# MachinePerceptionLab/Attentive_DFPrior

Hardware: AMD Instinct MI355X
Metric: rendered rays/sec (64 samples/ray), Replica room0 (higher is better)
Workload: dtype f32 via f16x3 split (3 f16 MFMA products per f32 product: 22-bit products, f32 accumulate); 1 GPU; room0 640x480 render_img, 64 spp (48+16), synthetic box room, seed-0 random decoders, grids at the REFERENCE init (N(0,.01), high N(0,1e-4)); stage color, ray_batch_size 100000 (per-batch far clamp, rendered as one call with a depth maximum per 100 000-ray segment), ONE frame per step; samples_per_ray=64

## Files before the change

attentive_dfprior_amd/csrc/adfp_decode_g.h:

```cpp
#pragma once
#include "adfp_decode_h.h"

__host__ __device__ constexpr int unit16(int k) { return 16 * ((k & 7) >> 2) + 4 * (k >> 3) + (k & 3); }

template <int CDIM, int NOUT>
struct DecLayoutG {
    using F = DecLayout<CDIM, NOUT>;
    static constexpr int KG_E = 3;
    static constexpr int KG_C = CDIM / 32;
    __host__ __device__ static constexpr int kg(int i) { return i == 0 ? KG_E : (i == 3 ? KG_E + 1 : 1); }
    static constexpr int P_BM = 0;
    __host__ __device__ static constexpr int layer_words(int i) { return kg(i) * 1024 + 32 + KG_C * 1024 + 32; }
    __host__ __device__ static constexpr int P_WP(int i) {
        int o = 384;
        for (int k = 0; k < i; ++k) o += layer_words(k);
        return o;
    }
    __host__ __device__ static constexpr int P_BP(int i) { return P_WP(i) + kg(i) * 1024; }
    __host__ __device__ static constexpr int P_WC(int i) { return P_BP(i) + 32; }
    __host__ __device__ static constexpr int P_BC(int i) { return P_WC(i) + KG_C * 1024; }
    static constexpr int P_WO = P_WP(5);
    static constexpr int P_BO = P_WO + NOUT * 32;
    static constexpr int P_FLAG = P_BO + 4;
    static constexpr int NFLAG = (((P_FLAG + 511) / 256) + 3) & ~3;
    static constexpr int P_TOTAL = P_FLAG + NFLAG;
    static_assert((P_TOTAL + 255) / 256 <= NFLAG, "one flag word per pack block");
};

template <int CDIM, int NOUT>
__device__ HSrc dec_g_src(int t) {
    using L = DecLayoutG<CDIM, NOUT>;
    using F = DecLayout<CDIM, NOUT>;
    if (t < 384) {
        const int row = t >> 2, c = t & 3;
        const int f = (row & ~31) + unit16(row & 31);
        return HSrc{0, (f < 93 && c < 3) ? F::F_EB + c * 93 + f : -1, -1};
    }
#pragma unroll
    for (int i = 0; i < 5; ++i) {
        if (t < L::P_BP(i) || (t >= L::P_WC(i) && t < L::P_BC(i))) {
            const bool fc = t >= L::P_WC(i);
            const int u = t - (fc ? L::P_WC(i) : L::P_WP(i));
            const int grp = u >> 10, ob = (u >> 9) & 1, part = (u >> 8) & 1, g = (u >> 6) & 3, row = 16 * ob + ((u >> 2) & 15), jp = (u & 3) * 2;
            int src[2];
#pragma unroll
            for (int e = 0; e < 2; ++e) {
                int col = 32 * grp + unit16(8 * g + jp + e);
                if (fc) src[e] = F::F_FC(i) + row * CDIM + col;
                else {
                    if (i == 0) { if (col >= 93) col = -1; }
                    else if (i == 3) { if (col < 96) { if (col >= 93) col = -1; } else col = 93 + (col - 96); }
                    src[e] = col < 0 ? -1 : F::F_PL(i) + row * F::in_dim(i) + col;
                }
            }
            return HSrc{1 + part, src[0], src[1]};
        }
        if (t < L::P_WC(i)) return HSrc{0, F::F_PL(i) + 32 * F::in_dim(i) + (t - L::P_BP(i)), -1};
        if (t < L::P_BC(i) + 32) return HSrc{0, F::F_FC(i) + 32 * CDIM + (t - L::P_BC(i)), -1};
    }
    if (t < L::P_BO) {
        const int u = t - L::P_WO;
        return HSrc{0, F::F_OW + u, -1};
    }
    const int o = t - L::P_BO;
    return HSrc{0, o < NOUT ? F::F_OB + o : -1, -1};
}

template <int CDIM, int NOUT>
ADFP_DEV void pack_decoder_g_block(int blk, const float* __restrict__ flat, unsigned* __restrict__ packed, int* __restrict__ status, int bit) {
    using L = DecLayoutG<CDIM, NOUT>;
    const int t = blk * 256 + (int)threadIdx.x;
    HSrc s{0, -1, -1};
    float a = 0.f, b = 0.f;
    if (t < L::P_FLAG) {
        s = dec_g_src<CDIM, NOUT>(t);
        a = s.s0 < 0 ? 0.f : flat[s.s0]; b = s.s1 < 0 ? 0.f : flat[s.s1];
    }
    pack_block_flag(!(fmaxf(fabsf(a), fabsf(b)) < 65504.0f), packed + L::P_FLAG + blk, status, bit);
    if (t >= L::P_FLAG) return;
    if (s.kind == 0) { packed[t] = s.s0 < 0 ? 0u : __float_as_uint(a); return; }
    a = f16_clamp(a); b = f16_clamp(b);
    const float ah = f16_hi_part(a), bh = f16_hi_part(b);
    _Float16 x, y;
    if (s.kind == 1) { x = (_Float16)ah; y = (_Float16)bh; }
    else { x = (_Float16)(a - ah); y = (_Float16)(b - bh); }
    packed[t] = (unsigned)__builtin_bit_cast(unsigned short, x) | ((unsigned)__builtin_bit_cast(unsigned short, y) << 16);
}
template <int CDIM, int NOUT>
__global__ void k_pack_decoder_g(const float* __restrict__ flat, unsigned* __restrict__ packed, int* __restrict__ status, int bit) { pack_decoder_g_block<CDIM, NOUT>((int)blockIdx.x, flat, packed, status, bit); }

typedef float f32x4g __attribute__((ext_vector_type(4)));

ADFP_DEV void swap_halves(float& x, float& y) {
    const auto r = __builtin_amdgcn_permlane32_swap(__float_as_uint(x), __float_as_uint(y), false, false);
    x = __uint_as_float(r[0]); y = __uint_as_float(r[1]);
}

template <int NG>
ADFP_DEV void mfma_chain_g(f32x4g acc[2][2], const unsigned* __restrict__ w, const f16x8 (*xh)[2], const f16x8 (*xl)[2]) {
#pragma unroll
    for (int kg = 0; kg < NG; ++kg) {
#pragma unroll
        for (int ob = 0; ob < 2; ++ob) {
            const f16x8 ah = __builtin_bit_cast(f16x8, *(const u32x4*)(w + kg * 1024 + ob * 512));
            const f16x8 al = __builtin_bit_cast(f16x8, *(const u32x4*)(w + kg * 1024 + ob * 512 + 256));
#pragma unroll
            for (int pb = 0; pb < 2; ++pb) {
                acc[ob][pb] = __builtin_amdgcn_mfma_f32_16x16x32_f16(ah, xh[kg][pb], acc[ob][pb], 0, 0, 0);
                acc[ob][pb] = __builtin_amdgcn_mfma_f32_16x16x32_f16(ah, xl[kg][pb], acc[ob][pb], 0, 0, 0);
                acc[ob][pb] = __builtin_amdgcn_mfma_f32_16x16x32_f16(al, xh[kg][pb], acc[ob][pb], 0, 0, 0);
            }
        }
    }
    __builtin_amdgcn_sched_barrier(0);
}

ADFP_DEV void row_store(float* p, const f32x4 v) {
    *(f32x4*)p = v;
}
template <int CDIM, int NOUT, int TRAIN = 0>
ADFP_DEV void decode_net_g(const unsigned* __restrict__ ldsu, const GridDev& grid, const GridDev& grid1, const float pn[3], const float (*pf)[3],
                           int lane, float& amax, float (*out)[NOUT], unsigned* __restrict__ mw, float* srow0, unsigned rowbits) {
    using L = DecLayoutG<CDIM, NOUT>;
    using ST = DecStage<CDIM>;
    const int g = lane >> 4;
    float* srow[2] = {nullptr, nullptr};
    if constexpr (TRAIN) {
        srow[0] = (rowbits & 1u) ? srow0 : nullptr;
        srow[1] = (rowbits & 2u) ? srow0 + 16 * ST::NXM : nullptr;
    }
    const unsigned* wl = ldsu + 4 * lane;
    const float* b4 = (const float*)ldsu + 4 * g;
    const float* brow = (const float*)ldsu + 32 * g;
    f16x8 ch[L::KG_C][2], cl[L::KG_C][2];
#pragma unroll
    for (int kc = 0; kc < L::KG_C; ++kc) {
        float c[16];
        gather16(kc == 0 ? grid : grid1, pn, g & 1, c);
        float x[8] = {c[0], c[1], c[2], c[3], c[8], c[9], c[10], c[11]};
        float y[8] = {c[4], c[5], c[6], c[7], c[12], c[13], c[14], c[15]};
#pragma unroll
        for (int s = 0; s < 8; ++s) swap_halves(x[s], y[s]);
        if constexpr (TRAIN) {
            static_assert(!TRAIN || CDIM == 32, "training rows: 32-channel decoders");
            if (srow[0]) { row_store(srow[0] + ST::xm(ST::SC) + 4 * g, f32x4{x[0], x[1], x[2], x[3]}); row_store(srow[0] + ST::xm(ST::SC) + 16 + 4 * g, f32x4{x[4], x[5], x[6], x[7]}); }
            if (srow[1]) { row_store(srow[1] + ST::xm(ST::SC) + 4 * g, f32x4{y[0], y[1], y[2], y[3]}); row_store(srow[1] + ST::xm(ST::SC) + 16 + 4 * g, f32x4{y[4], y[5], y[6], y[7]}); }
        }
        split8(x, ch[kc][0], cl[kc][0], amax);
        split8(y, ch[kc][1], cl[kc][1], amax);
    }
    f16x8 eh[L::KG_E][2], el[L::KG_E][2];
#pragma unroll
    for (int kg = 0; kg < L::KG_E; ++kg) {
        float e0[8], e1[8];
#pragma unroll
        for (int j = 0; j < 8; ++j) {
            const f32x4 bm = *(const f32x4*)(brow + L::P_BM + (32 * kg + j) * 4);
            e0[j] = adfp_sinf(fmaf(pf[0][2], bm.z, fmaf(pf[0][1], bm.y, pf[0][0] * bm.x)));
            e1[j] = adfp_sinf(fmaf(pf[1][2], bm.z, fmaf(pf[1][1], bm.y, pf[1][0] * bm.x)));
        }
        split8<false>(e0, eh[kg][0], el[kg][0], amax);
        split8<false>(e1, eh[kg][1], el[kg][1], amax);
    }
    __builtin_amdgcn_sched_barrier(0);
    f32x4g acc[2][2];
    f16x8 hh[1][2], hl[1][2];
    unsigned mk[3] = {0u, 0u, 0u};
#pragma unroll
    for (int i = 0; i < 5; ++i) {
#pragma unroll
        for (int ob = 0; ob < 2; ++ob) { const f32x4 t = *(const f32x4*)(b4 + L::P_BP(i) + 16 * ob); acc[ob][0] = t; acc[ob][1] = t; }
        if (i == 0) mfma_chain_g<L::KG_E>(acc, wl + L::P_WP(0), eh, el);
        else if (i == 3) {
            mfma_chain_g<L::KG_E>(acc, wl + L::P_WP(3), eh, el);
            mfma_chain_g<1>(acc, wl + L::P_WP(3) + L::KG_E * 1024, hh, hl);
        } else mfma_chain_g<1>(acc, wl + L::P_WP(i), hh, hl);
#pragma unroll
        for (int ob = 0; ob < 2; ++ob) {
            const f32x4 t = *(const f32x4*)(b4 + L::P_BC(i) + 16 * ob);
#pragma unroll
            for (int pb = 0; pb < 2; ++pb)
#pragma unroll
                for (int r = 0; r < 4; ++r) {
                    const float v = relu_f(acc[ob][pb][r]);
                    if constexpr (TRAIN) mk[i >> 1] = __builtin_amdgcn_alignbit(mk[i >> 1], 0u - __float_as_uint(v), 31);
                    acc[ob][pb][r] = v + t[r];
                }
        }
        mfma_chain_g<L::KG_C>(acc, wl + L::P_WC(i), ch, cl);
        if constexpr (TRAIN) {
#pragma unroll
            for (int pb = 0; pb < 2; ++pb) if (srow[pb]) {
                row_store(srow[pb] + ST::xm(ST::SH(i)) + 4 * g, f32x4{acc[0][pb][0], acc[0][pb][1], acc[0][pb][2], acc[0][pb][3]});
                row_store(srow[pb] + ST::xm(ST::SH(i)) + 16 + 4 * g, f32x4{acc[1][pb][0], acc[1][pb][1], acc[1][pb][2], acc[1][pb][3]});
            }
        }
        if (i < 4) {
#pragma unroll
            for (int pb = 0; pb < 2; ++pb) {
                const float t[8] = {acc[0][pb][0], acc[0][pb][1], acc[0][pb][2], acc[0][pb][3],
                                    acc[1][pb][0], acc[1][pb][1], acc[1][pb][2], acc[1][pb][3]};
                split8(t, hh[0][pb], hl[0][pb], amax);
            }
        }
    }
#pragma unroll
    for (int o = 0; o < NOUT; ++o) {
        const f32x4 w0 = *(const f32x4*)(b4 + L::P_WO + 32 * o), w1 = *(const f32x4*)(b4 + L::P_WO + 32 * o + 16);
#pragma unroll
        for (int pb = 0; pb < 2; ++pb) {
            float s = 0.f;
#pragma unroll
            for (int r = 0; r < 4; ++r) s = fmaf(acc[0][pb][r], w0[r], s);
#pragma unroll
            for (int r = 0; r < 4; ++r) s = fmaf(acc[1][pb][r], w1[r], s);
            s += __shfl_xor(s, 16);
            s += __shfl_xor(s, 32);
            out[pb][o] = s + ((const float*)ldsu)[L::P_BO + o];
        }
    }
    if constexpr (TRAIN) {
        const int sh = 4 * (g >> 1);
        unsigned wpb[2][3];
#pragma unroll
        for (int pb = 0; pb < 2; ++pb) {
            unsigned f[5];
#pragma unroll
            for (int i = 0; i < 5; ++i) {
                const unsigned m16 = (i == 4 || (i & 1)) ? (mk[i >> 1] & 0xFFFFu) : (mk[i >> 1] >> 16);
                const unsigned n0 = (m16 >> (12 - 4 * pb)) & 0xFu, n1 = (m16 >> (4 - 4 * pb)) & 0xFu;
                f[i] = (n0 << (12 - sh)) | (n1 << (4 - sh));
            }
            wpb[pb][0] = f[0] | (f[1] << 16); wpb[pb][1] = f[2] | (f[3] << 16); wpb[pb][2] = f[4];
        }
#pragma unroll
        for (int k = 0; k < 3; ++k) {
            const auto r = __builtin_amdgcn_permlane32_swap(wpb[0][k], wpb[1][k], false, false);
            mw[k] = r[0] | r[1];
        }
    }
}

template <int NT>
__global__ __launch_bounds__(NT, NT / 256) void k_decode_lc16(DecodeLCArgs a) {
    using LL = DecLayoutG<32, 1>;
    using LC = DecLayoutG<32, 4>;
    __shared__ __attribute__((aligned(16))) unsigned lds_all[LL::P_TOTAL + LC::P_TOTAL];
    __shared__ int s_next;
    __shared__ unsigned long long s_ring[ADFP_POOL_RING];
    unsigned* lds_low = lds_all;
    unsigned* lds_col = lds_all + LL::P_TOTAL;
    image_to_lds<NT, LL::P_TOTAL / 4>(lds_low, a.packed_low);
    image_to_lds<NT, LC::P_TOTAL / 4>(lds_col, a.packed_color);
    if (threadIdx.x == 0) s_next = NT / 64;
    if (threadIdx.x < ADFP_POOL_RING) s_ring[threadIdx.x] = 0ull;
    __syncthreads();
    const int lane = threadIdx.x & 63, n = lane & 15, g = lane >> 4;
    const int count = a.P.n;
    const int ntiles = (count + 31) >> 5;
    const TilePlan plan = tile_plan(ntiles, (int)gridDim.x, NT / 64, a.pool != nullptr);
    float amax_low = image_out_of_range<LL::P_FLAG, LL::NFLAG>(lds_low) ? INFINITY : 0.f;
    float amax_col = image_out_of_range<LC::P_FLAG, LC::NFLAG>(lds_col) ? INFINITY : 0.f;
    for (int j = threadIdx.x >> 6, tile; (tile = claim_tile_pool<NT / 64>(j, &s_next, s_ring, plan, ntiles, a.pool, a.status)) >= 0;) {
        const int idx = tile * 32 + 16 * (g >> 1) + n;
        const bool valid = idx < count;
        const int q = valid ? idx : 0;
        float pn[3], pf[2][3];
        bool pnan, keep_occ;
        {
            double pt[3];
            load_point(a.P, q, pt);
            normalize3(a.nb, pt, pn);
            const float f0 = (float)pt[0], f1 = (float)pt[1], f2 = (float)pt[2];
            pnan = (pt[0] != pt[0]) | (pt[1] != pt[1]) | (pt[2] != pt[2]);
            const unsigned f = a.flags ? a.flags[q] : 0u;
            keep_occ = (f & ADFP_F_BAND) || in_bound(pt, a.b) || !a.apply_bound;
            pf[0][0] = f0; pf[0][1] = f1; pf[0][2] = f2; pf[1][0] = f0; pf[1][1] = f1; pf[1][2] = f2;
        }
#pragma unroll
        for (int k = 0; k < 3; ++k) swap_halves(pf[0][k], pf[1][k]);
        float occ[2][1], rgb[2][4];
        int off_low = 0, off_col = LL::P_TOTAL;
        asm volatile("" : "+v"(off_low), "+v"(off_col));
        decode_net_g<32, 1>(lds_all + off_low, a.g_low, a.g_low, pn, pf, lane, amax_low, occ, nullptr, nullptr, 0u);
        asm volatile("" : "+v"(pn[0]), "+v"(pn[1]), "+v"(pn[2]), "+v"(occ[0][0]), "+v"(occ[1][0]));
        __builtin_amdgcn_sched_barrier(0);
        decode_net_g<32, 4>(lds_all + off_col, a.g_color, a.g_color, pn, pf, lane, amax_col, rgb, nullptr, nullptr, 0u);
        if (valid && (g & 1) == 0) {
            const int pb = g >> 1;
            const float nanv = __builtin_nanf("");
            const float o = pnan ? nanv : (keep_occ ? (pb ? occ[1][0] : occ[0][0]) : 100.f);
            const f32x4 c4 = pb ? f32x4{rgb[1][0], rgb[1][1], rgb[1][2], o} : f32x4{rgb[0][0], rgb[0][1], rgb[0][2], o};
            *(f32x4*)(a.raw + 4ll * q) = pnan ? f32x4{nanv, nanv, nanv, o} : c4;
            if (a.write_w) a.w[q] = 1.f;
        }
    }
    report_range(a.status, amax_low, ADFP_STATUS_F16_RANGE_LOW, a.call_flag);
    report_range(a.status, amax_col, ADFP_STATUS_F16_RANGE_COLOR, a.call_flag);
}

struct DecodeLCTrainArgs {
    DecodeLCArgs f;
    unsigned* masks_low; unsigned* masks_color;
    float* act_low; float* act_color;
    int split_networks;
};
template <int NT, bool SPLIT = false>
__global__ __launch_bounds__(NT, NT / 256) void k_decode_lc16_train(DecodeLCTrainArgs t) {
    const DecodeLCArgs& a = t.f;
    using LL = DecLayoutG<32, 1>;
    using LC = DecLayoutG<32, 4>;
    using ST = DecStage<32>;
    __shared__ __attribute__((aligned(16))) unsigned lds_all[LL::P_TOTAL + LC::P_TOTAL];
    __shared__ int s_next;
    unsigned* lds_low = lds_all;
    unsigned* lds_col = lds_all + LL::P_TOTAL;
    image_to_lds<NT, LL::P_TOTAL / 4>(lds_low, a.packed_low);
    image_to_lds<NT, LC::P_TOTAL / 4>(lds_col, a.packed_color);
    if (threadIdx.x == 0) s_next = NT / 64;
    __syncthreads();
    const int lane = threadIdx.x & 63, n = lane & 15, g = lane >> 4;
    const int count = a.P.n;
    const int ntiles = (count + 31) >> 5;
    float amax_low = image_out_of_range<LL::P_FLAG, LL::NFLAG>(lds_low) ? INFINITY : 0.f;
    float amax_col = image_out_of_range<LC::P_FLAG, LC::NFLAG>(lds_col) ? INFINITY : 0.f;
    constexpr bool split = SPLIT;
    const int njobs = split ? 2 * ntiles : ntiles;
    for (int j = threadIdx.x >> 6, job; (job = claim_tile<NT / 64>(j, &s_next, njobs)) >= 0;) {
        const int tile = split ? job >> 1 : job;
        const bool do_low = !split || (job & 1) == 0, do_col = !split || (job & 1) == 1;
        const int idx = tile * 32 + 16 * (g >> 1) + n;
        const bool valid = idx < count;
        const int q = valid ? idx : 0;
        float pn[3], pf[2][3];
        bool pnan, keep_occ;
        {
            double pt[3];
            load_point(a.P, q, pt);
            normalize3(a.nb, pt, pn);
            pnan = (pt[0] != pt[0]) | (pt[1] != pt[1]) | (pt[2] != pt[2]);
            const float f0 = pnan ? 0.f : (float)pt[0], f1 = pnan ? 0.f : (float)pt[1], f2 = pnan ? 0.f : (float)pt[2];
            const unsigned f = a.flags ? a.flags[q] : 0u;
            keep_occ = (f & ADFP_F_BAND) || in_bound(pt, a.b) || !a.apply_bound;
            pf[0][0] = f0; pf[0][1] = f1; pf[0][2] = f2; pf[1][0] = f0; pf[1][1] = f1; pf[1][2] = f2;
        }
#pragma unroll
        for (int k = 0; k < 3; ++k) swap_halves(pf[0][k], pf[1][k]);
        const int i0 = tile * 32 + n;
        const unsigned rowbits = (i0 < count ? 1u : 0u) | (i0 + 16 < count ? 2u : 0u);
        float occ[2][1], rgb[2][4];
        unsigned mw[3];
        int off_low = 0, off_col = LL::P_TOTAL;
        asm volatile("" : "+v"(off_low), "+v"(off_col));
        if constexpr (split) {
            occ[0][0] = 0.f; occ[1][0] = 0.f;
#pragma unroll
            for (int k = 0; k < 4; ++k) { rgb[0][k] = 0.f; rgb[1][k] = 0.f; }
        }
        if (do_low) {
            decode_net_g<32, 1, 1>(lds_all + off_low, a.g_low, a.g_low, pn, pf, lane, amax_low, occ, mw, t.act_low + (long long)i0 * ST::NXM, t.act_low ? rowbits : 0u);
            if (valid) { unsigned* mrow = t.masks_low + ((long long)q * 2 + (g & 1)) * 3; mrow[0] = mw[0]; mrow[1] = mw[1]; mrow[2] = mw[2]; }
        }
        asm volatile("" : "+v"(pn[0]), "+v"(pn[1]), "+v"(pn[2]), "+v"(occ[0][0]), "+v"(occ[1][0]));
        __builtin_amdgcn_sched_barrier(0);
        if (do_col) {
            decode_net_g<32, 4, 1>(lds_all + off_col, a.g_color, a.g_color, pn, pf, lane, amax_col, rgb, mw, t.act_color + (long long)i0 * ST::NXM, t.act_color ? rowbits : 0u);
            if (valid) { unsigned* mrow = t.masks_color + ((long long)q * 2 + (g & 1)) * 3; mrow[0] = mw[0]; mrow[1] = mw[1]; mrow[2] = mw[2]; }
        }
        if (valid && (g & 1) == 0) {
            const int pb = g >> 1;
            const float nanv = __builtin_nanf("");
            const float o = pnan ? nanv : (keep_occ ? (pb ? occ[1][0] : occ[0][0]) : 100.f);
            const f32x4 c4 = pb ? f32x4{rgb[1][0], rgb[1][1], rgb[1][2], o} : f32x4{rgb[0][0], rgb[0][1], rgb[0][2], o};
            const f32x4 row = pnan ? f32x4{nanv, nanv, nanv, o} : c4;
            if (!split) {
                *(f32x4*)(a.raw + 4ll * q) = row;
                if (a.write_w) a.w[q] = 1.f;
            } else if (do_low) {
                a.raw[4ll * q + 3] = row.w;
                if (a.write_w) a.w[q] = 1.f;
            } else {
                a.raw[4ll * q] = row.x; a.raw[4ll * q + 1] = row.y; a.raw[4ll * q + 2] = row.z;
            }
        }
    }
    report_range(a.status, amax_low, ADFP_STATUS_F16_RANGE_LOW, a.call_flag);
    report_range(a.status, amax_col, ADFP_STATUS_F16_RANGE_COLOR, a.call_flag);
}

template <int NT>
__global__ __launch_bounds__(NT, NT / 256) void k_decode_high_g(DecodeArgs a) {
    using L = DecLayoutG<64, 1>;
    __shared__ __attribute__((aligned(16))) unsigned ldsu[L::P_TOTAL];
    __shared__ int s_next;
    __shared__ unsigned long long s_ring[ADFP_POOL_RING];
    image_to_lds<NT, L::P_TOTAL / 4>(ldsu, a.packed);
    if (threadIdx.x == 0) s_next = NT / 64;
    if (threadIdx.x < ADFP_POOL_RING) s_ring[threadIdx.x] = 0ull;
    __syncthreads();
    const int lane = threadIdx.x & 63, n = lane & 15, g = lane >> 4;
    const int count = *a.count_ptr;
    const int ntiles = (count + 31) >> 5;
    const TilePlan plan = tile_plan(ntiles, (int)gridDim.x, NT / 64, a.pool != nullptr);
    float amax = image_out_of_range<L::P_FLAG, L::NFLAG>(ldsu) ? INFINITY : 0.f;
    for (int j = threadIdx.x >> 6, tile; (tile = claim_tile_pool<NT / 64>(j, &s_next, s_ring, plan, ntiles, a.pool, a.status)) >= 0;) {
        const int idx = tile * 32 + 16 * (g >> 1) + n;
        const bool valid = idx < count;
        const int q = a.list[valid ? idx : 0];
        float pn[3], pf[2][3];
        bool pnan;
        const float low_occ = (a.single || !valid) ? 0.f : a.raw[4ll * q + 3];
        {
            double pt[3];
            load_point(a.P, q, pt);
            normalize3(a.nb, pt, pn);
            const float f0 = (float)pt[0], f1 = (float)pt[1], f2 = (float)pt[2];
            pnan = (pt[0] != pt[0]) | (pt[1] != pt[1]) | (pt[2] != pt[2]);
            pf[0][0] = f0; pf[0][1] = f1; pf[0][2] = f2; pf[1][0] = f0; pf[1][1] = f1; pf[1][2] = f2;
        }
#pragma unroll
        for (int k = 0; k < 3; ++k) swap_halves(pf[0][k], pf[1][k]);
        float out[2][1];
        decode_net_g<64, 1>(ldsu, a.g0, a.g1, pn, pf, lane, amax, out, nullptr, nullptr, 0u);
        if (valid && (g & 1) == 0) {
            const float o = g >> 1 ? out[1][0] : out[0][0];
            const float v = pnan ? __builtin_nanf("") : o;
            a.att_occ[idx] = a.single ? v : v + low_occ;
        }
    }
    report_range(a.status, amax, ADFP_STATUS_F16_RANGE_HIGH, a.call_flag);
}

struct AttLayoutG {
    using F = AttLayout;
    static constexpr int P_A0 = 0;
    static constexpr int P_W1 = 256;
    static constexpr int P_B1 = P_W1 + 4 * 2 * 1024;
    static constexpr int P_W2 = P_B1 + 128;
    static constexpr int P_B2 = P_W2 + 4 * 4 * 1024;
    static constexpr int P_W3 = P_B2 + 128;
    static constexpr int P_B3 = P_W3 + 2 * 4 * 1024;
    static constexpr int P_WO = P_B3 + 64;
    static constexpr int P_BO = P_WO + 128;
    static constexpr int P_FLAG = P_BO + 4;
    static constexpr int NFLAG = (((P_FLAG + 511) / 256) + 3) & ~3;
    static constexpr int P_TOTAL = P_FLAG + NFLAG;
    static_assert((P_TOTAL + 255) / 256 <= NFLAG, "one flag word per pack block");
};

__device__ HSrc att_g_src(int t) {
    using L = AttLayoutG;
    using F = AttLayout;
    if (t < L::P_W1) {
        const int row = t >> 2, c = t & 3;
        const int u = (row & ~31) + unit16(row & 31);
        return HSrc{0, c < 2 ? F::F_W0 + u * 2 + c : (c == 2 ? F::F_B0 + u : -1), -1};
    }
    auto chain = [](int u, int ngrp, int base, int ld) {
        const int blk = u / (ngrp * 1024), v = u % (ngrp * 1024);
        const int grp = v >> 10, ob = (v >> 9) & 1, part = (v >> 8) & 1, g = (v >> 6) & 3, row = 32 * blk + 16 * ob + ((v >> 2) & 15), jp = (v & 3) * 2;
        return HSrc{1 + part, base + row * ld + 32 * grp + unit16(8 * g + jp), base + row * ld + 32 * grp + unit16(8 * g + jp + 1)};
    };
    if (t < L::P_B1) return chain(t - L::P_W1, 2, F::F_W1, 64);
    if (t < L::P_W2) return HSrc{0, F::F_B1 + (t - L::P_B1), -1};
    if (t < L::P_B2) return chain(t - L::P_W2, 4, F::F_W2, 128);
    if (t < L::P_W3) return HSrc{0, F::F_B2 + (t - L::P_B2), -1};
    if (t < L::P_B3) return chain(t - L::P_W3, 4, F::F_W3, 128);
    if (t < L::P_WO) return HSrc{0, F::F_B3 + (t - L::P_B3), -1};
    if (t < L::P_BO) return HSrc{0, F::F_WO + (t - L::P_WO), -1};
    const int o = t - L::P_BO;
    return HSrc{0, o < 2 ? F::F_BO + o : -1, -1};
}

ADFP_DEV void pack_attention_g_block(int blk, const float* __restrict__ flat, unsigned* __restrict__ packed, int* __restrict__ status) {
    using L = AttLayoutG;
    const int t = blk * 256 + (int)threadIdx.x;
    HSrc s{0, -1, -1};
    float a = 0.f, b = 0.f;
    if (t < L::P_FLAG) {
        s = att_g_src(t);
        a = s.s0 < 0 ? 0.f : flat[s.s0]; b = s.s1 < 0 ? 0.f : flat[s.s1];
    }
    pack_block_flag(!(fmaxf(fabsf(a), fabsf(b)) < 65504.0f), packed + L::P_FLAG + blk, status, ADFP_STATUS_F16_RANGE_ATT);
    if (t >= L::P_FLAG) return;
    if (s.kind == 0) { packed[t] = s.s0 < 0 ? 0u : __float_as_uint(a); return; }
    a = f16_clamp(a); b = f16_clamp(b);
    const float ah = f16_hi_part(a), bh = f16_hi_part(b);
    _Float16 x, y;
    if (s.kind == 1) { x = (_Float16)ah; y = (_Float16)bh; }
    else { x = (_Float16)(a - ah); y = (_Float16)(b - bh); }
    packed[t] = (unsigned)__builtin_bit_cast(unsigned short, x) | ((unsigned)__builtin_bit_cast(unsigned short, y) << 16);
}
__global__ void k_pack_attention_g(const float* __restrict__ flat, unsigned* __restrict__ packed, int* __restrict__ status) { pack_attention_g_block((int)blockIdx.x, flat, packed, status); }

template <int NT>
__global__ __launch_bounds__(NT) void k_attention_g(AttArgs a) {
    using A = AttLayoutG;
    __shared__ __attribute__((aligned(16))) unsigned ldsu[A::P_TOTAL];
    __shared__ int s_next;
    __shared__ unsigned long long s_ring[ADFP_POOL_RING];
    image_to_lds<NT, A::P_TOTAL / 4>(ldsu, a.packed);
    if (threadIdx.x == 0) s_next = NT / 64;
    if (threadIdx.x < ADFP_POOL_RING) s_ring[threadIdx.x] = 0ull;
    __syncthreads();
    const float* lds = (const float*)ldsu;
    const int lane = threadIdx.x & 63, n = lane & 15, g = lane >> 4;
    const unsigned* wl = ldsu + 4 * lane;
    const float* b4 = lds + 4 * g;
    const float* arow = lds + 32 * g;
    const int count = a.count_ptr ? *a.count_ptr : a.n_rows;
    const int ntiles = (count + 31) >> 5;
    const TilePlan plan = tile_plan(ntiles, (int)gridDim.x, NT / 64, a.pool != nullptr);
    float amax = image_out_of_range<A::P_FLAG, A::NFLAG>(ldsu) ? INFINITY : 0.f;
    for (int j = threadIdx.x >> 6, tile; (tile = claim_tile_pool<NT / 64>(j, &s_next, s_ring, plan, ntiles, a.pool, a.status)) >= 0;) {
        int idx[2]; bool valid[2]; float occ[2], u[2];
#pragma unroll
        for (int pb = 0; pb < 2; ++pb) {
            idx[pb] = tile * 32 + 16 * pb + n;
            valid[pb] = idx[pb] < count;
            const int ii = valid[pb] ? idx[pb] : 0;
            occ[pb] = a.att_occ[ii]; u[pb] = a.att_u[ii];
        }
        f16x8 xh[4][2], xl[4][2];
#pragma unroll
        for (int b = 0; b < 2; ++b) {
            float t0[8], t1[8];
#pragma unroll
            for (int k = 0; k < 8; ++k) {
                const f32x4 t = *(const f32x4*)(arow + A::P_A0 + (32 * b + k) * 4);
                t0[k] = relu_f(fmaf(u[0], t.y, fmaf(occ[0], t.x, t.z)));
                t1[k] = relu_f(fmaf(u[1], t.y, fmaf(occ[1], t.x, t.z)));
            }
            split8(t0, xh[b][0], xl[b][0], amax);
            split8(t1, xh[b][1], xl[b][1], amax);
        }
        __builtin_amdgcn_sched_barrier(0);
        f16x8 yh[4][2], yl[4][2];
#pragma unroll
        for (int blk = 0; blk < 4; ++blk) {
            f32x4g acc[2][2];
#pragma unroll
            for (int ob = 0; ob < 2; ++ob) { const f32x4 t = *(const f32x4*)(b4 + A::P_B1 + 32 * blk + 16 * ob); acc[ob][0] = t; acc[ob][1] = t; }
            mfma_chain_g<2>(acc, wl + A::P_W1 + blk * 2 * 1024, xh, xl);
#pragma unroll
            for (int pb = 0; pb < 2; ++pb) {
                const float t[8] = {relu_f(acc[0][pb][0]), relu_f(acc[0][pb][1]), relu_f(acc[0][pb][2]), relu_f(acc[0][pb][3]),
                                    relu_f(acc[1][pb][0]), relu_f(acc[1][pb][1]), relu_f(acc[1][pb][2]), relu_f(acc[1][pb][3])};
                split8(t, yh[blk][pb], yl[blk][pb], amax);
            }
        }
#pragma unroll
        for (int blk = 0; blk < 4; ++blk) {
            f32x4g acc[2][2];
#pragma unroll
            for (int ob = 0; ob < 2; ++ob) { const f32x4 t = *(const f32x4*)(b4 + A::P_B2 + 32 * blk + 16 * ob); acc[ob][0] = t; acc[ob][1] = t; }
            mfma_chain_g<4>(acc, wl + A::P_W2 + blk * 4 * 1024, yh, yl);
#pragma unroll
            for (int pb = 0; pb < 2; ++pb) {
                const float t[8] = {relu_f(acc[0][pb][0]), relu_f(acc[0][pb][1]), relu_f(acc[0][pb][2]), relu_f(acc[0][pb][3]),
                                    relu_f(acc[1][pb][0]), relu_f(acc[1][pb][1]), relu_f(acc[1][pb][2]), relu_f(acc[1][pb][3])};
                split8(t, xh[blk][pb], xl[blk][pb], amax);
            }
        }
        float l0[2] = {0.f, 0.f}, l1[2] = {0.f, 0.f};
#pragma unroll
        for (int blk = 0; blk < 2; ++blk) {
            f32x4g acc[2][2];
#pragma unroll
            for (int ob = 0; ob < 2; ++ob) { const f32x4 t = *(const f32x4*)(b4 + A::P_B3 + 32 * blk + 16 * ob); acc[ob][0] = t; acc[ob][1] = t; }
            mfma_chain_g<4>(acc, wl + A::P_W3 + blk * 4 * 1024, xh, xl);
#pragma unroll
            for (int ob = 0; ob < 2; ++ob) {
                const f32x4 w0 = *(const f32x4*)(b4 + A::P_WO + 32 * blk + 16 * ob), w1 = *(const f32x4*)(b4 + A::P_WO + 64 + 32 * blk + 16 * ob);
#pragma unroll
                for (int pb = 0; pb < 2; ++pb)
#pragma unroll
                    for (int r = 0; r < 4; ++r) {
                        const float v = relu_f(acc[ob][pb][r]);
                        l0[pb] = fmaf(v, w0[r], l0[pb]);
                        l1[pb] = fmaf(v, w1[r], l1[pb]);
                    }
            }
        }
#pragma unroll
        for (int pb = 0; pb < 2; ++pb) {
            l0[pb] += __shfl_xor(l0[pb], 16); l0[pb] += __shfl_xor(l0[pb], 32);
            l1[pb] += __shfl_xor(l1[pb], 16); l1[pb] += __shfl_xor(l1[pb], 32);
        }
        if (g < 2 && valid[g]) {
            const float a0l = l0[g] + lds[A::P_BO], a1l = l1[g] + lds[A::P_BO + 1];
            const float m = fmaxf(a0l, a1l);
            const float e0 = expf(a0l - m), e1 = expf(a1l - m);
            const float den = e0 + e1;
            const float a0 = e0 / den, a1 = e1 / den;
            const float fused = a0 * occ[g] + a1 * u[g];
            const int ii = idx[g];
            const int q = a.list ? a.list[ii] : ii;
            const bool inb = !a.flags || (a.flags[q] & ADFP_F_INBOUND) != 0;
            a.raw[4ll * q + 3] = (inb || !a.apply_bound) ? fused : 100.f;
            a.w[q] = a1;
        }
    }
    report_range(a.status, amax, ADFP_STATUS_F16_RANGE_ATT, a.call_flag);
}
```

Measured before the change: 58.87 million rays/s.

## Software-pipeline high decoder and attention MLP chains with interleaved LDS reads and MFMA

Adds a hand-scheduled high-band decoder (decode_net_gp) that double-buffers weight operand reads from LDS and interleaves the Fourier feature computation, ReLU and f16 splitting with MFMA chains, using sched_group_barrier slots. The attention kernel is rewritten into one flattened 10-chunk chain. It prefetches the next chunk's weights and the next tile's inputs while the current MFMAs run, and spreads the previous chunk's epilogue (split or output dot) between MFMAs. The aim is to hide LDS latency and VALU epilogue work behind matrix ops, at the cost of higher register pressure and fragile compiler scheduling.

```diff
diff --git a/attentive_dfprior_amd/csrc/adfp_decode_g.h b/attentive_dfprior_amd/csrc/adfp_decode_g.h
--- a/attentive_dfprior_amd/csrc/adfp_decode_g.h
+++ b/attentive_dfprior_amd/csrc/adfp_decode_g.h
@@ -388,6 +388,210 @@
     report_range(a.status, amax_col, ADFP_STATUS_F16_RANGE_COLOR, a.call_flag);
 }
 
+struct AOpG { u32x4 h[2], l[2]; };
+ADFP_DEV void aop_read(AOpG& A, const unsigned* __restrict__ w, int ob) {
+    A.h[ob] = *(const u32x4*)(w + ob * 512);
+    A.l[ob] = *(const u32x4*)(w + ob * 512 + 256);
+}
+ADFP_DEV void mfma6_g(f32x4g acc[2], const u32x4 ah, const u32x4 al, const u32x4 xh[2], const u32x4 xl[2]) {
+    const f16x8 h = __builtin_bit_cast(f16x8, ah), l = __builtin_bit_cast(f16x8, al);
+    const f16x8 h0 = __builtin_bit_cast(f16x8, xh[0]), h1 = __builtin_bit_cast(f16x8, xh[1]);
+    const f16x8 l0 = __builtin_bit_cast(f16x8, xl[0]), l1 = __builtin_bit_cast(f16x8, xl[1]);
+    acc[0] = __builtin_amdgcn_mfma_f32_16x16x32_f16(h, h0, acc[0], 0, 0, 0);
+    acc[1] = __builtin_amdgcn_mfma_f32_16x16x32_f16(h, h1, acc[1], 0, 0, 0);
+    acc[0] = __builtin_amdgcn_mfma_f32_16x16x32_f16(h, l0, acc[0], 0, 0, 0);
+    acc[1] = __builtin_amdgcn_mfma_f32_16x16x32_f16(h, l1, acc[1], 0, 0, 0);
+    acc[0] = __builtin_amdgcn_mfma_f32_16x16x32_f16(l, h0, acc[0], 0, 0, 0);
+    acc[1] = __builtin_amdgcn_mfma_f32_16x16x32_f16(l, h1, acc[1], 0, 0, 0);
+}
+ADFP_DEV void split_pair(float a, float b, unsigned& hi, unsigned& lo, float& amax, unsigned m1) {
+    typedef _Float16 h2 __attribute__((ext_vector_type(2)));
+    const h2 neg1 = __builtin_bit_cast(h2, m1);
+    amax = __builtin_fmaxf(__builtin_fmaxf(__builtin_fabsf(a), __builtin_fabsf(b)), amax);
+    asm volatile("" : "+v"(amax));
+    const h2 hp = __builtin_bit_cast(h2, __builtin_amdgcn_cvt_pkrtz(a, b));
+    h2 lp;
+    lp[0] = (_Float16)__builtin_fmaf((float)hp[0], (float)neg1[0], a);
+    lp[1] = (_Float16)__builtin_fmaf((float)hp[1], (float)neg1[0], b);
+    hi = __builtin_bit_cast(unsigned, hp);
+    lo = __builtin_bit_cast(unsigned, lp);
+}
+#define ADFP_SLOT_END()                                                      \
+    do {                                                                     \
+        __builtin_amdgcn_sched_group_barrier(0x100, 2, 0);                   \
+        for (int s_ = 0; s_ < 6; ++s_) {                                     \
+            __builtin_amdgcn_sched_group_barrier(0x008, 1, 0);               \
+            __builtin_amdgcn_sched_group_barrier(0x002, 2, 0);               \
+        }                                                                    \
+        __builtin_amdgcn_sched_barrier(0);                                   \
+    } while (0)
+
+ADFP_DEV void mfma6_pb(f32x4g acc[2][2], int pb, const AOpG& A, const u32x4 xh, const u32x4 xl) {
+    const f16x8 h0 = __builtin_bit_cast(f16x8, A.h[0]), h1 = __builtin_bit_cast(f16x8, A.h[1]);
+    const f16x8 l0 = __builtin_bit_cast(f16x8, A.l[0]), l1 = __builtin_bit_cast(f16x8, A.l[1]);
+    const f16x8 bh = __builtin_bit_cast(f16x8, xh), bl = __builtin_bit_cast(f16x8, xl);
+    acc[0][pb] = __builtin_amdgcn_mfma_f32_16x16x32_f16(h0, bh, acc[0][pb], 0, 0, 0);
+    acc[1][pb] = __builtin_amdgcn_mfma_f32_16x16x32_f16(h1, bh, acc[1][pb], 0, 0, 0);
+    acc[0][pb] = __builtin_amdgcn_mfma_f32_16x16x32_f16(h0, bl, acc[0][pb], 0, 0, 0);
+    acc[1][pb] = __builtin_amdgcn_mfma_f32_16x16x32_f16(h1, bl, acc[1][pb], 0, 0, 0);
+    acc[0][pb] = __builtin_amdgcn_mfma_f32_16x16x32_f16(l0, bh, acc[0][pb], 0, 0, 0);
+    acc[1][pb] = __builtin_amdgcn_mfma_f32_16x16x32_f16(l1, bh, acc[1][pb], 0, 0, 0);
+}
+template <bool CHECK = true>
+ADFP_DEV void split8u(const float* __restrict__ x, u32x4& hi, u32x4& lo, float& amax) {
+    f16x8 h, l;
+    split8<CHECK>(x, h, l, amax);
+    hi = __builtin_bit_cast(u32x4, h); lo = __builtin_bit_cast(u32x4, l);
+}
+#define ADFP_SLOT(NDS, NM, NV)                                               \
+    do {                                                                     \
+        __builtin_amdgcn_sched_group_barrier(0x100, NDS, 0);                 \
+        for (int s_ = 0; s_ < NM; ++s_) {                                    \
+            __builtin_amdgcn_sched_group_barrier(0x008, 1, 0);               \
+            __builtin_amdgcn_sched_group_barrier(0x002, NV, 0);              \
+        }                                                                    \
+        __builtin_amdgcn_sched_barrier(0);                                   \
+    } while (0)
+
+template <int CDIM, int NOUT>
+ADFP_DEV void decode_net_gp(const unsigned* __restrict__ ldsu, const GridDev& grid, const GridDev& grid1, const float pn[3], const float (*pf)[3],
+                            int lane, float& amax, float (*out)[NOUT]) {
+    using L = DecLayoutG<CDIM, NOUT>;
+    static_assert(L::KG_C == 2 && L::KG_E == 3, "the in-band decoder: own grid + low grid, 96 Fourier rows");
+    const int g = lane >> 4;
+    const unsigned* wl = ldsu + 4 * lane;
+    const float* b4 = (const float*)ldsu + 4 * g;
+    const float* brow = (const float*)ldsu + 32 * g;
+    AOpG P[2], Q[2];
+    auto rd = [&](AOpG& A, const int woff) { aop_read(A, wl + woff, 0); aop_read(A, wl + woff, 1); };
+    auto rdb = [&](f32x4 (&b)[2], const int off) { b[0] = *(const f32x4*)(b4 + off); b[1] = *(const f32x4*)(b4 + off + 16); };
+    f32x4 bp[2], bc[2];
+    rd(P[0], L::P_WP(0));
+    rdb(bp, L::P_BP(0));
+    u32x4 ch[2][2], cl[2][2];
+#pragma unroll
+    for (int kc = 0; kc < 2; ++kc) {
+        float c[16];
+        gather16(kc == 0 ? grid : grid1, pn, g & 1, c);
+        float x[8] = {c[0], c[1], c[2], c[3], c[8], c[9], c[10], c[11]};
+        float y[8] = {c[4], c[5], c[6], c[7], c[12], c[13], c[14], c[15]};
+#pragma unroll
+        for (int s = 0; s < 8; ++s) swap_halves(x[s], y[s]);
+        split8u(x, ch[kc][0], cl[kc][0], amax);
+        split8u(y, ch[kc][1], cl[kc][1], amax);
+    }
+    u32x4 eh[3][2], el[3][2];
+    auto feat = [&](const int kg) {
+        float e0[8], e1[8];
+#pragma unroll
+        for (int j = 0; j < 8; ++j) {
+            const f32x4 bm = *(const f32x4*)(brow + L::P_BM + (32 * kg + j) * 4);
+            e0[j] = adfp_sinf(fmaf(pf[0][2], bm.z, fmaf(pf[0][1], bm.y, pf[0][0] * bm.x)));
+            e1[j] = adfp_sinf(fmaf(pf[1][2], bm.z, fmaf(pf[1][1], bm.y, pf[1][0] * bm.x)));
+        }
+        split8u<false>(e0, eh[kg][0], el[kg][0], amax);
+        split8u<false>(e1, eh[kg][1], el[kg][1], amax);
+    };
+    feat(0);
+    f32x4g acc[2][2], acc3[2][2];
+    u32x4 hh[2], hl[2];
+#pragma unroll
+    for (int ob = 0; ob < 2; ++ob) { acc[ob][0] = bp[ob]; acc[ob][1] = bp[ob]; }
+    __builtin_amdgcn_sched_barrier(0);
+    auto F = [&](f32x4g (&a)[2][2], const AOpG& A, const int ob, const int kg) { mfma6_g(a[ob], A.h[ob], A.l[ob], eh[kg], el[kg]); };
+    auto R = [&](const int pb) {
+#pragma unroll
+        for (int ob = 0; ob < 2; ++ob)
+#pragma unroll
+            for (int r = 0; r < 4; ++r) acc[ob][pb][r] = relu_f(acc[ob][pb][r]) + bc[ob][r];
+    };
+    auto C = [&](const int pb) { mfma6_pb(acc, pb, Q[0], ch[0][pb], cl[0][pb]); mfma6_pb(acc, pb, Q[1], ch[1][pb], cl[1][pb]); };
+    auto S = [&](const int pb) {
+        const float t[8] = {acc[0][pb][0], acc[0][pb][1], acc[0][pb][2], acc[0][pb][3], acc[1][pb][0], acc[1][pb][1], acc[1][pb][2], acc[1][pb][3]};
+        split8u(t, hh[pb], hl[pb], amax);
+    };
+    rd(P[1], L::P_WP(0) + 1024);
+    F(acc, P[0], 0, 0); F(acc, P[0], 1, 0);
+    feat(1);
+    ADFP_SLOT(12, 12, 8);
+    rd(P[0], L::P_WP(0) + 2048);
+    F(acc, P[1], 0, 1); F(acc, P[1], 1, 1);
+    feat(2);
+    ADFP_SLOT(12, 12, 8);
+    rd(P[1], L::P_WP(3));
+    rdb(bc, L::P_BC(0));
+    rdb(bp, L::P_BP(3));
+    F(acc, P[0], 0, 2); F(acc, P[0], 1, 2);
+    ADFP_SLOT(8, 12, 0);
+#pragma unroll
+    for (int ob = 0; ob < 2; ++ob) { acc3[ob][0] = bp[ob]; acc3[ob][1] = bp[ob]; }
+    rd(Q[0], L::P_WC(0)); rd(Q[1], L::P_WC(0) + 1024);
+    F(acc3, P[1], 0, 0); F(acc3, P[1], 1, 0);
+    R(0); R(1);
+    ADFP_SLOT(8, 12, 3);
+    rd(P[0], L::P_WP(1));
+    C(0);
+    ADFP_SLOT(4, 12, 0);
+    rd(P[1], L::P_WP(3) + 1024);
+    rdb(bp, L::P_BP(1));
+    C(1);
+    S(0);
+    ADFP_SLOT(6, 12, 2);
+#pragma unroll
+    for (int i = 1; i < 5; ++i) {
+        const bool fill = i < 3;
+        rd(Q[0], L::P_WC(i));
+        rdb(bc, L::P_BC(i));
+        if (i == 3) {
+#pragma unroll
+            for (int ob = 0; ob < 2; ++ob) acc[ob][0] = acc3[ob][0];
+        } else {
+#pragma unroll
+            for (int ob = 0; ob < 2; ++ob) acc[ob][0] = bp[ob];
+        }
+        mfma6_pb(acc, 0, P[0], hh[0], hl[0]);
+        if (fill) F(acc3, P[1], 0, i);
+        S(1);
+        if (fill) ADFP_SLOT(6, 12, 2); else ADFP_SLOT(6, 6, 4);
+        rd(Q[1], L::P_WC(i) + 1024);
+        if (i == 3) {
+#pragma unroll
+            for (int ob = 0; ob < 2; ++ob) acc[ob][1] = acc3[ob][1];
+        } else {
+#pragma unroll
+            for (int ob = 0; ob < 2; ++ob) acc[ob][1] = bp[ob];
+        }
+        mfma6_pb(acc, 1, P[0], hh[1], hl[1]);
+        if (fill) F(acc3, P[1], 1, i);
+        R(0);
+        if (fill) ADFP_SLOT(4, 12, 2); else ADFP_SLOT(4, 6, 3);
+        if (i < 4) rd(P[0], i == 2 ? L::P_WP(3) + 3 * 1024 : L::P_WP(i + 1));
+        if (i < 4 && i != 2) rdb(bp, L::P_BP(i + 1));
+        C(0);
+        R(1);
+        ADFP_SLOT(6, 12, 2);
+        if (i == 1) rd(P[1], L::P_WP(3) + 2 * 1024);
+        C(1);
+        if (i < 4) S(0);
+        ADFP_SLOT(4, 12, 2);
+    }
+#pragma unroll
+    for (int o = 0; o < NOUT; ++o) {
+        const f32x4 w0 = *(const f32x4*)(b4 + L::P_WO + 32 * o), w1 = *(const f32x4*)(b4 + L::P_WO + 32 * o + 16);
+#pragma unroll
+        for (int pb = 0; pb < 2; ++pb) {
+            float s = 0.f;
+#pragma unroll
+            for (int r = 0; r < 4; ++r) s = fmaf(acc[0][pb][r], w0[r], s);
+#pragma unroll
+            for (int r = 0; r < 4; ++r) s = fmaf(acc[1][pb][r], w1[r], s);
+            s += __shfl_xor(s, 16);
+            s += __shfl_xor(s, 32);
+            out[pb][o] = s + ((const float*)ldsu)[L::P_BO + o];
+        }
+    }
+}
+
 template <int NT>
 __global__ __launch_bounds__(NT, NT / 256) void k_decode_high_g(DecodeArgs a) {
     using L = DecLayoutG<64, 1>;
@@ -421,7 +625,7 @@
 #pragma unroll
         for (int k = 0; k < 3; ++k) swap_halves(pf[0][k], pf[1][k]);
         float out[2][1];
-        decode_net_g<64, 1>(ldsu, a.g0, a.g1, pn, pf, lane, amax, out, nullptr, nullptr, 0u);
+        decode_net_gp<64, 1>(ldsu, a.g0, a.g1, pn, pf, lane, amax, out);
         if (valid && (g & 1) == 0) {
             const float o = g >> 1 ? out[1][0] : out[0][0];
             const float v = pnan ? __builtin_nanf("") : o;
@@ -493,9 +697,20 @@
 }
 __global__ void k_pack_attention_g(const float* __restrict__ flat, unsigned* __restrict__ packed, int* __restrict__ status) { pack_attention_g_block((int)blockIdx.x, flat, packed, status); }
 
+struct AttChainG {
+    using A = AttLayoutG;
+    __host__ __device__ static constexpr int layer(int c) { return c < 4 ? 1 : (c < 8 ? 2 : 3); }
+    __host__ __device__ static constexpr int blk(int c) { return c & 3; }
+    __host__ __device__ static constexpr int ng(int c) { return c < 4 ? 2 : 4; }
+    __host__ __device__ static constexpr int w(int c) { return c < 4 ? A::P_W1 + c * 2 * 1024 : (c < 8 ? A::P_W2 + (c - 4) * 4 * 1024 : A::P_W3 + (c - 8) * 4 * 1024); }
+    __host__ __device__ static constexpr int b(int c) { return c < 4 ? A::P_B1 + 32 * c : (c < 8 ? A::P_B2 + 32 * (c - 4) : A::P_B3 + 32 * (c - 8)); }
+    __host__ __device__ static constexpr int step0(int c) { return c < 4 ? 2 * c : 8 + 4 * (c - 4); }
+};
+
 template <int NT>
 __global__ __launch_bounds__(NT) void k_attention_g(AttArgs a) {
     using A = AttLayoutG;
+    using C = AttChainG;
     __shared__ __attribute__((aligned(16))) unsigned ldsu[A::P_TOTAL];
     __shared__ int s_next;
     __shared__ unsigned long long s_ring[ADFP_POOL_RING];
@@ -512,16 +727,32 @@
     const int ntiles = (count + 31) >> 5;
     const TilePlan plan = tile_plan(ntiles, (int)gridDim.x, NT / 64, a.pool != nullptr);
     float amax = image_out_of_range<A::P_FLAG, A::NFLAG>(ldsu) ? INFINITY : 0.f;
-    for (int j = threadIdx.x >> 6, tile; (tile = claim_tile_pool<NT / 64>(j, &s_next, s_ring, plan, ntiles, a.pool, a.status)) >= 0;) {
-        int idx[2]; bool valid[2]; float occ[2], u[2];
+    auto fetch = [&](const int t, float (&o)[2], float (&v)[2]) {
+#pragma unroll
+        for (int pb = 0; pb < 2; ++pb) {
+            const int i = t * 32 + 16 * pb + n, ii = i < count ? i : 0;
+            o[pb] = a.att_occ[ii]; v[pb] = a.att_u[ii];
+        }
+    };
+    int j = threadIdx.x >> 6;
+    int tile = claim_tile_pool<NT / 64>(j, &s_next, s_ring, plan, ntiles, a.pool, a.status);
+    float occ_n[2] = {0.f, 0.f}, u_n[2] = {0.f, 0.f};
+    if (tile >= 0) fetch(tile, occ_n, u_n);
+    while (tile >= 0) {
+        int idx[2]; bool valid[2];
+        const float occ[2] = {occ_n[0], occ_n[1]}, u[2] = {u_n[0], u_n[1]};
 #pragma unroll
         for (int pb = 0; pb < 2; ++pb) {
             idx[pb] = tile * 32 + 16 * pb + n;
             valid[pb] = idx[pb] < count;
-            const int ii = valid[pb] ? idx[pb] : 0;
-            occ[pb] = a.att_occ[ii]; u[pb] = a.att_u[ii];
-        }
-        f16x8 xh[4][2], xl[4][2];
+        }
+        const int tile_next = claim_tile_pool<NT / 64>(j, &s_next, s_ring, plan, ntiles, a.pool, a.status);
+        if (tile_next >= 0) fetch(tile_next, occ_n, u_n);
+        AOpG aop[2];
+        aop_read(aop[0], wl + C::w(0), 0);
+        aop_read(aop[0], wl + C::w(0), 1);
+        f32x4 bias[2] = {*(const f32x4*)(b4 + C::b(0)), *(const f32x4*)(b4 + C::b(0) + 16)};
+        u32x4 xh[4][2], xl[4][2];
 #pragma unroll
         for (int b = 0; b < 2; ++b) {
             float t0[8], t1[8];
@@ -531,57 +762,66 @@
                 t0[k] = relu_f(fmaf(u[0], t.y, fmaf(occ[0], t.x, t.z)));
                 t1[k] = relu_f(fmaf(u[1], t.y, fmaf(occ[1], t.x, t.z)));
             }
-            split8(t0, xh[b][0], xl[b][0], amax);
-            split8(t1, xh[b][1], xl[b][1], amax);
-        }
+            f16x8 h0, l0, h1, l1;
+            split8(t0, h0, l0, amax);
+            split8(t1, h1, l1, amax);
+            xh[b][0] = __builtin_bit_cast(u32x4, h0); xl[b][0] = __builtin_bit_cast(u32x4, l0);
+            xh[b][1] = __builtin_bit_cast(u32x4, h1); xl[b][1] = __builtin_bit_cast(u32x4, l1);
+        }
+        unsigned m1 = 0xBC00BC00u;
+        asm volatile("" : "+v"(m1));
+        u32x4 yh[4][2], yl[4][2];
+        f32x4g acc[2][2][2];
+        f32x4 wo[2][2];
+        float l0[2] = {0.f, 0.f}, l1[2] = {0.f, 0.f};
+#pragma unroll
+        for (int ob = 0; ob < 2; ++ob) { acc[0][ob][0] = bias[ob]; acc[0][ob][1] = bias[ob]; }
         __builtin_amdgcn_sched_barrier(0);
-        f16x8 yh[4][2], yl[4][2];
-#pragma unroll
-        for (int blk = 0; blk < 4; ++blk) {
-            f32x4g acc[2][2];
-#pragma unroll
-            for (int ob = 0; ob < 2; ++ob) { const f32x4 t = *(const f32x4*)(b4 + A::P_B1 + 32 * blk + 16 * ob); acc[ob][0] = t; acc[ob][1] = t; }
-            mfma_chain_g<2>(acc, wl + A::P_W1 + blk * 2 * 1024, xh, xl);
-#pragma unroll
-            for (int pb = 0; pb < 2; ++pb) {
-                const float t[8] = {relu_f(acc[0][pb][0]), relu_f(acc[0][pb][1]), relu_f(acc[0][pb][2]), relu_f(acc[0][pb][3]),
-                                    relu_f(acc[1][pb][0]), relu_f(acc[1][pb][1]), relu_f(acc[1][pb][2]), relu_f(acc[1][pb][3])};
-                split8(t, yh[blk][pb], yl[blk][pb], amax);
+        auto piece = [&](const int c, const int p) {
+            const int ob = p >> 2, pb = (p >> 1) & 1, r = 2 * (p & 1), w = 2 * ob + (p & 1);
+            const float v0 = relu_f(acc[c & 1][ob][pb][r]), v1 = relu_f(acc[c & 1][ob][pb][r + 1]);
+            if (C::layer(c) < 3) {
+                unsigned hi, lo;
+                split_pair(v0, v1, hi, lo, amax, m1);
+                if (C::layer(c) == 1) { yh[C::blk(c)][pb][w] = hi; yl[C::blk(c)][pb][w] = lo; }
+                else { xh[C::blk(c)][pb][w] = hi; xl[C::blk(c)][pb][w] = lo; }
+            } else {
+                l0[pb] = fmaf(v0, wo[0][ob][r], l0[pb]); l1[pb] = fmaf(v0, wo[1][ob][r], l1[pb]);
+                l0[pb] = fmaf(v1, wo[0][ob][r + 1], l0[pb]); l1[pb] = fmaf(v1, wo[1][ob][r + 1], l1[pb]);
             }
-        }
-#pragma unroll
-        for (int blk = 0; blk < 4; ++blk) {
-            f32x4g acc[2][2];
-#pragma unroll
-            for (int ob = 0; ob < 2; ++ob) { const f32x4 t = *(const f32x4*)(b4 + A::P_B2 + 32 * blk + 16 * ob); acc[ob][0] = t; acc[ob][1] = t; }
-            mfma_chain_g<4>(acc, wl + A::P_W2 + blk * 4 * 1024, yh, yl);
-#pragma unroll
-            for (int pb = 0; pb < 2; ++pb) {
-                const float t[8] = {relu_f(acc[0][pb][0]), relu_f(acc[0][pb][1]), relu_f(acc[0][pb][2]), relu_f(acc[0][pb][3]),
-                                    relu_f(acc[1][pb][0]), relu_f(acc[1][pb][1]), relu_f(acc[1][pb][2]), relu_f(acc[1][pb][3])};
-                split8(t, xh[blk][pb], xl[blk][pb], amax);
+        };
+#pragma unroll
+        for (int c = 0; c < 10; ++c) {
+            const int NG = C::ng(c);
+#pragma unroll
+            for (int kg = 0; kg < 4; ++kg) {
+                if (kg < NG) {
+                    const int step = C::step0(c) + kg, cur = step & 1;
+                    const int cn = kg + 1 < NG ? c : c + 1, kn = kg + 1 < NG ? kg + 1 : 0;
+#pragma unroll
+                    for (int ob = 0; ob < 2; ++ob) {
+                        const int si = 2 * kg + ob, last = 2 * NG - 1;
+                        if (cn < 10) aop_read(aop[cur ^ 1], wl + C::w(cn) + kn * 1024, ob);
+                        if (C::layer(c) == 2) mfma6_g(acc[c & 1][ob], aop[cur].h[ob], aop[cur].l[ob], yh[kg], yl[kg]);
+                        else mfma6_g(acc[c & 1][ob], aop[cur].h[ob], aop[cur].l[ob], xh[kg], xl[kg]);
+                        if (c > 0 && si < 4) { piece(c - 1, 2 * si); piece(c - 1, 2 * si + 1); }
+                        if (si == last - 1 && c < 9) { bias[0] = *(const f32x4*)(b4 + C::b(c + 1)); bias[1] = *(const f32x4*)(b4 + C::b(c + 1) + 16); }
+                        if (C::layer(c) == 3 && si >= 4 && si < 6) {
+                            const int o = si - 4;
+                            wo[o][0] = *(const f32x4*)(b4 + A::P_WO + 64 * o + 32 * C::blk(c));
+                            wo[o][1] = *(const f32x4*)(b4 + A::P_WO + 64 * o + 32 * C::blk(c) + 16);
+                        }
+                        if (si == last && c < 9) {
+#pragma unroll
+                            for (int o2 = 0; o2 < 2; ++o2) { acc[(c + 1) & 1][o2][0] = bias[o2]; acc[(c + 1) & 1][o2][1] = bias[o2]; }
+                        }
+                        ADFP_SLOT_END();
+                    }
+                }
             }
         }
-        float l0[2] = {0.f, 0.f}, l1[2] = {0.f, 0.f};
-#pragma unroll
-        for (int blk = 0; blk < 2; ++blk) {
-            f32x4g acc[2][2];
-#pragma unroll
-            for (int ob = 0; ob < 2; ++ob) { const f32x4 t = *(const f32x4*)(b4 + A::P_B3 + 32 * blk + 16 * ob); acc[ob][0] = t; acc[ob][1] = t; }
-            mfma_chain_g<4>(acc, wl + A::P_W3 + blk * 4 * 1024, xh, xl);
-#pragma unroll
-            for (int ob = 0; ob < 2; ++ob) {
-                const f32x4 w0 = *(const f32x4*)(b4 + A::P_WO + 32 * blk + 16 * ob), w1 = *(const f32x4*)(b4 + A::P_WO + 64 + 32 * blk + 16 * ob);
-#pragma unroll
-                for (int pb = 0; pb < 2; ++pb)
-#pragma unroll
-                    for (int r = 0; r < 4; ++r) {
-                        const float v = relu_f(acc[ob][pb][r]);
-                        l0[pb] = fmaf(v, w0[r], l0[pb]);
-                        l1[pb] = fmaf(v, w1[r], l1[pb]);
-                    }
-            }
-        }
+#pragma unroll
+        for (int p = 0; p < 8; ++p) piece(9, p);
 #pragma unroll
         for (int pb = 0; pb < 2; ++pb) {
             l0[pb] += __shfl_xor(l0[pb], 16); l0[pb] += __shfl_xor(l0[pb], 32);
@@ -600,6 +840,7 @@
             a.raw[4ll * q + 3] = (inb || !a.apply_bound) ? fused : 100.f;
             a.w[q] = a1;
         }
+        tile = tile_next;
     }
     report_range(a.status, amax, ADFP_STATUS_F16_RANGE_ATT, a.call_flag);
 }
```

After: 59.37 million rays/s, median of 6. No clear change (+0.9%).
